# tangih/video-matting

Measured on AMD Instinct MI355X. Metric: alpha-mattes/sec at 1920×1080, 1/2/4/8 MI355X + achieved HBM GB/s, higher is better.
Workload: dtype bf16; 1 GPU; unet.UNetVideo forward (20 3x3 convs, 3.233 TFLOP/frame), 1920x1080 7-ch NHWC; height=1080, width=1920, launch=hip-graph replay, parallelism=frame-parallel dp1

## Files before the change

### video-matting_amd/csrc/conv3x3.hip

```cpp

#include <cstring>
#include <initializer_list>

#include "conv_dispatch.h"

namespace vm {


struct TileOrigin {
  int h0, w0;
  float rcp_w, rcp_h;
};

__device__ __forceinline__ TileOrigin tile_origin(long m0, int H, int W) {
  TileOrigin o;
  const long q = m0 / W;
  o.w0 = (int)(m0 - q * W);
  o.h0 = (int)(q % H);
  o.rcp_w = __builtin_amdgcn_rcpf((float)W);
  o.rcp_h = __builtin_amdgcn_rcpf((float)H);
  return o;
}

__device__ __forceinline__ int fast_div(int t, int d, float rcp) {
// ... 454 lines not shown
        float bsv[4] = {0.f, 0.f, 0.f, 0.f}, scv[4] = {1.f, 1.f, 1.f, 1.f}, shv[4] = {0.f, 0.f, 0.f, 0.f};
#pragma unroll
        for (int j = 0; j < 4; ++j) {
          const int co = min(n0 + wn * 64 + col + j, a.cout - 1);
          if (a.bias) bsv[j] = a.bias[co];
          if (a.scale) scv[j] = a.scale[co];
          if (a.shift) shv[j] = a.shift[co];
        }
#pragma unroll
        for (int fp = 0; fp < FP; ++fp) {
          const int row = wm * C::TPM + fp * 16 + (lane & 15);
          float4 v;
          float* vv = reinterpret_cast<float*>(&v);
#pragma unroll
          for (int j = 0; j < 4; ++j) {
            float tv = (acc[fc][fp][j] + bsv[j]) * scv[j] + shv[j];
            if (a.act == VM_ACT_RELU) tv = tv > 0.f ? tv : 0.f;
            else if (a.act == VM_ACT_SIGMOID) tv = sigmoid_precise(tv);
            vv[j] = tv;
          }
          *reinterpret_cast<float4*>(stg + row * SROW + col) = v;
        }
      }
    }
    __syncthreads();
    const int nb = n0 + sl * 64;
    if (a.y_dtype == VM_BF16) {
      uint16_t* Y = reinterpret_cast<uint16_t*>(a.y) + a.y_coff;
      for (int idx = tid; idx < BM * 8; idx += NT) {
        const int rr = idx >> 3, cc = idx & 7;
        const long p = m0 + rr;
        const int co = nb + cc * 8;
        if (p >= a.M || co >= a.cout) continue;
        const float* src = stg + rr * SROW + cc * 8;
        uint16_t* dst = Y + p * (long)a.y_cstride + co;
        if (a.y_vec && co + 8 <= a.cout) *reinterpret_cast<uint4*>(dst) = Chunk<uint16_t>::pack(src);
        else
          for (int j = 0; j < 8 && co + j < a.cout; ++j) dst[j] = f2bf(src[j]);
      }
    } else {
      float* Y = reinterpret_cast<float*>(a.y) + a.y_coff;
      for (int idx = tid; idx < BM * 16; idx += NT) {
        const int rr = idx >> 4, cc = idx & 15;
        const long p = m0 + rr;
        const int co = nb + cc * 4;
        if (p >= a.M || co >= a.cout) continue;
        const float* src = stg + rr * SROW + cc * 4;
        float* dst = Y + p * (long)a.y_cstride + co;
        if (a.y_vec && co + 4 <= a.cout) *reinterpret_cast<float4*>(dst) = *reinterpret_cast<const float4*>(src);
        else
          for (int j = 0; j < 4 && co + j < a.cout; ++j) dst[j] = src[j];
      }
    }
  }
}

thread_local char g_last_kernel[128];
ConvOptions g_opt;
template <typename T>
static const char* tname() { return sizeof(T) == 2 ? "unsigned short" : "float"; }

template <typename T, int BM, int BN>
static int launch_mfma(ConvArgs& a, hipStream_t st) {
  constexpr int lds = mfma_lds_bytes<BM, BN>();
  static bool attr_set = false;
  if (!attr_set) {
    hipError_t e = hipFuncSetAttribute(reinterpret_cast<const void*>(&conv3x3_mfma<T, BM, BN>),
                                       hipFuncAttributeMaxDynamicSharedMemorySize, lds);
    if (e != hipSuccess) return fail(VM_EHIP, "hipFuncSetAttribute: %s", hipGetErrorString(e));
    attr_set = true;
  }
  a.nk = a.K_pad / (128 / (int)sizeof(T));
  a.tiles_n = (a.cout + BN - 1) / BN;
  a.tiles_total = (int)((a.M + BM - 1) / BM) * a.tiles_n;
  snprintf(g_last_kernel, sizeof g_last_kernel, "vm::conv3x3_mfma<%s, %d, %d>", tname<T>(), BM, BN);
  hipLaunchKernelGGL((conv3x3_mfma<T, BM, BN>), dim3(a.tiles_total), dim3(256), lds, st, a);
  return check_launch("conv3x3_mfma");
}

template <typename T, int RB, int BM, int BN, int WM, int WN, int S, bool FAST>
static int launch_glds(ConvArgs& a, hipStream_t st) {
  using C = GldsCfg<T, RB, BM, BN, WM, WN, S>;
  static bool attr_set = false;
  if (!attr_set) {
    hipError_t e = hipFuncSetAttribute(reinterpret_cast<const void*>(&conv3x3_glds<T, RB, BM, BN, WM, WN, S, FAST>),
                                       hipFuncAttributeMaxDynamicSharedMemorySize, C::LDS);
    if (e != hipSuccess) return fail(VM_EHIP, "hipFuncSetAttribute(glds): %s", hipGetErrorString(e));
    attr_set = true;
  }
  const int bke = RB / (int)sizeof(T);
  a.nk = (FAST && RB == 64) ? a.ng : a.K_pad / bke;
  a.tiles_n = (a.cout + BN - 1) / BN;
  a.tiles_total = (int)((a.M + BM - 1) / BM) * a.tiles_n;
  snprintf(g_last_kernel, sizeof g_last_kernel, "vm::conv3x3_glds<%s, %d, %d, %d, %d, %d, %d, %s>", tname<T>(), RB,
           BM, BN, WM, WN, S, FAST ? "true" : "false");
  hipLaunchKernelGGL((conv3x3_glds<T, RB, BM, BN, WM, WN, S, FAST>), dim3(a.tiles_total), dim3(C::NT), C::LDS, st,
                     a);
  return check_launch("conv3x3_glds");
}

template <typename T, bool FAST>
static int dispatch_glds(ConvArgs& a, hipStream_t st) {
  if constexpr (sizeof(T) == 2) {
    if (a.cout > 128) {
      if (g_opt.glds_rb == 64) return launch_glds<T, 64, 256, 256, 2, 4, 4, FAST>(a, st);
      return launch_glds<T, 128, 256, 256, 2, 4, 2, FAST>(a, st);
    }
  }
  if (a.cout > 64) return launch_glds<T, 64, 256, 128, 4, 2, 6, FAST>(a, st);
  return launch_glds<T, 64, 512, 64, 8, 1, 4, FAST>(a, st);
}

template <typename T>
static int dispatch_mfma(ConvArgs& a, hipStream_t st, int cin = 0) {
  if (sizeof(T) == 4 && g_opt.softmax_kernel != 0 && g_opt.conv_kernel != 1 && g_opt.conv_kernel != 2 && cin > 0 && cin <= 8 &&
      a.cin_pad == 8 && !a.chunk_major && a.x_src_c <= 0 && a.y_dtype == VM_F32 && a.y_vec && a.act == VM_ACT_SOFTMAX &&
      a.cout == 64 && a.K_pad == 96 && a.x_cstride % 4 == 0 && a.x_coff % 4 == 0 &&
      reinterpret_cast<uintptr_t>(a.x) % 16 == 0)
    return launch_first_softmax_f32(a, cin, st);
  if (sizeof(T) == 2 && g_opt.softmax_kernel != 0 && g_opt.conv_kernel != 1 && g_opt.conv_kernel != 2 && a.cin_pad == 8 &&
      !a.chunk_major && a.x_src_c <= 0 && a.y_dtype == VM_F32 && a.y_vec && a.act == VM_ACT_SOFTMAX && a.cout == 64 &&
      a.K_pad == 128)
    return launch_first_softmax(a, st);
  if (sizeof(T) == 2 && g_opt.conv_kernel != 1 && g_opt.conv_kernel != 2 && a.cin_pad == 8 && !a.chunk_major && a.x_src_c <= 0 &&
      a.y_dtype == VM_BF16 && a.y_vec && a.act != VM_ACT_SOFTMAX && (a.cout & 7) == 0 && a.K_pad == 128)
    return launch_first(a, st);
  if ((g_opt.conv_kernel == 0 || g_opt.conv_kernel == 3) && patch_ok(a, sizeof(T))) return dispatch_patch(a, st);
  if (g_opt.conv_kernel != 1 && a.act != VM_ACT_SOFTMAX && a.x_src_c <= 0) {
    const int bm = a.cout > 64 ? 256 : 512;
    const long tiles = ((a.M + bm - 1) / bm) * ((a.cout + 255) / 256);
    const bool wide = sizeof(T) == 2 && a.cout > 128;
    if (g_opt.conv_kernel == 2 || (wide && tiles >= g_opt.conv_min_tiles))
      return a.chunk_major ? dispatch_glds<T, true>(a, st) : dispatch_glds<T, false>(a, st);
  }
  if (a.cout <= 64) return launch_mfma<T, 256, 64>(a, st);
  return launch_mfma<T, 128, 128>(a, st);
}

static const OptDef conv_options[] = {
    {"conv_kernel", &g_opt.conv_kernel, OPT_RANGE, 2, {0, 3}},
    {"softmax_kernel", &g_opt.softmax_kernel, OPT_RANGE, 2, {0, 6}},
    {"softmax_blocks", &g_opt.softmax_blocks, OPT_RANGE, 2, {1, 1 << 20}},
    {"head_th", &g_opt.head_th, OPT_SET, 2, {8, 16}},
    {"softmax_f32p", &g_opt.softmax_f32p, OPT_RANGE, 2, {0, 7}},
    {"cband", &g_opt.cband, OPT_RANGE, 2, {0, 2}},
    {"ngroup", &g_opt.ngroup, OPT_RANGE, 2, {0, 64}},
    {"cband_bytes", &g_opt.cband_bytes, OPT_ANY},
    {"rows_kernel", &g_opt.rows_kernel, OPT_SET, 4, {0, 1, 8, 16}},
    {"pack_tiled", &g_opt.pack_tiled, OPT_ANY},
    {"persist_half", &g_opt.persist_half, OPT_ANY},
    {"rows_up", &g_opt.rows_up, OPT_ANY},
    {"rows_min_cin", &g_opt.rows_min_cin, OPT_ANY},
    {"rows_min_blocks", &g_opt.rows_min_blocks, OPT_ANY},
    {"thin_rounds", &g_opt.thin_rounds, OPT_RANGE, 2, {0, 64}},
    {"pack_frames", &g_opt.pack_frames, OPT_RANGE, 2, {0, 1}},
    {"up_skip", &g_opt.up_skip, OPT_RANGE, 2, {0, 1}},
    {"src_span_limit", &g_opt.src_span_limit, OPT_RANGE, 2, {1, 0x7ffffff0L}},
    {"thin_blocks", &g_opt.thin_blocks, OPT_ANY},
    {"thin_th", &g_opt.thin_th, OPT_SET, 3, {4, 8, 16}},
    {"conv_prio", &g_opt.conv_prio, OPT_RANGE, 2, {0, 1}},
    {"thin_twalk", &g_opt.thin_twalk, OPT_RANGE, 2, {0, 1}},
    {"thin_rowreuse", &g_opt.thin_rowreuse, OPT_RANGE, 2, {0, 1}},
    {"thin_dma", &g_opt.thin_dma, OPT_RANGE, 2, {0, 4}},
    {"thin_dma_rounds", &g_opt.thin_dma_rounds, OPT_RANGE, 2, {1, 64}},
    {"narrowin_kernel", &g_opt.narrowin_kernel, OPT_RANGE, 2, {0, 1}},
    {"thin_kernel", &g_opt.thin_kernel, OPT_RANGE, 2, {0, 1}},
    {"conv_min_tiles", &g_opt.conv_min_tiles, OPT_ANY},
#ifdef VM_STUDY
    {"patch_cfg", &g_opt.patch_cfg, OPT_RANGE, 2, {0, 31}},
    {"patch_ablate", &g_opt.patch_ablate, OPT_ANY},
    {"softmax_abl", &g_opt.softmax_abl, OPT_ANY},
    {"patch_rowslot", &g_opt.patch_rowslot, OPT_RANGE, 2, {0, 1}},
    {"pair_strip_abl", &g_opt.pair_strip_abl, OPT_ANY},
    {"pair_kernel", &g_opt.pair_kernel, OPT_RANGE, 2, {0, 1}},
    {"pair_kernel", &g_opt.pair_kernel, OPT_RANGE, 2, {10, 18}},
#else
    {"patch_cfg", &g_opt.patch_cfg, OPT_SET, 5, {0, 19, 22, 25, 30}, " (other tilings: the study build)"},
    {"pair_kernel", &g_opt.pair_kernel, OPT_RANGE, 2, {0, 1}, " (ablations: the study build)"},
#endif
    {"pair_xin_wide", &g_opt.pair_xin_wide, OPT_RANGE, 2, {0, 1}},
    {"border_ks", &g_opt.border_ks, OPT_SET, 3, {1, 2, 4}},
    {"border_fuse", &g_opt.border_fuse, OPT_RANGE, 2, {0, 2}},
    {"patch_repi", &g_opt.patch_repi, OPT_RANGE, 2, {0, 1}},
    {"persist_rounds", &g_opt.persist_rounds, OPT_RANGE, 2, {0, 64}, " (0: any grid)"},
    {"persist_up_rounds", &g_opt.persist_up_rounds, OPT_RANGE, 2, {0, 64}, " (0: any grid)"},
    {"persist_all", &g_opt.persist_all, OPT_RANGE, 2, {0, 2}},
    {"persist_rot", &g_opt.persist_rot, OPT_RANGE, 2, {0, 2}},
    {"up_skip_mask", &g_opt.up_skip_mask, OPT_RANGE, 2, {0, 3}},
    {"patch_persist", &g_opt.patch_persist, OPT_RANGE, 2, {0, 1}},
    {"pair_strip_pin", &g_opt.pair_strip_pin, OPT_RANGE, 2, {0, 1}},
    {"pair_strip", &g_opt.pair_strip, OPT_RANGE, 2, {0, 1}},
    {"head_kernel", &g_opt.head_kernel, OPT_RANGE, 2, {0, 2}},
    {"splitk_tiles", &g_opt.splitk_tiles, OPT_ANY},
    {"glds_rb", &g_opt.glds_rb, OPT_SET, 2, {64, 128}},
    {nullptr},
};
}

using namespace vm;

static int set_from(const OptDef* t, const char* key, long value) {
  char want[160] = "";
  const char* note = "";
  for (; t->key; ++t) {
    if (strcmp(key, t->key)) continue;
    bool ok = t->kind == OPT_ANY || (t->kind == OPT_RANGE && value >= t->v[0] && value <= t->v[1]);
    for (int i = 0; t->kind == OPT_SET && i < t->n; ++i) ok = ok || value == t->v[i];
    if (ok) {
      *t->value = value;
      return VM_OK;
    }
    size_t len = strlen(want);
    if (len) len += snprintf(want + len, sizeof want - len, " or ");
    if (t->kind == OPT_RANGE) snprintf(want + len, sizeof want - len, "%ld..%ld", t->v[0], t->v[1]);
    for (int i = 0; t->kind == OPT_SET && i < t->n && len < sizeof want; ++i)
      len += snprintf(want + len, sizeof want - len, i == 0 ? "%ld" : i + 1 < t->n ? ", %ld" : " or %ld", t->v[i]);
    if (t->note) note = t->note;
  }
  return want[0] ? fail(VM_EINVAL, "set_option: %s must be %s%s", key, want, note) : 1;
}

extern "C" int vm_set_option(const char* key, long value) {
  if (!key) return fail(VM_EINVAL, "set_option: NULL key");
  for (const OptDef* t : {conv_options, bn_options, train_options, wgrad_options, flow_options}) {
    const int rc = set_from(t, key, value);
    if (rc != 1) return rc;
  }
  return fail(VM_EINVAL, "set_option: unknown key '%s'", key);
}

extern "C" const char* vm_conv3x3_last_kernel(void) { return g_last_kernel; }

static int conv_impl(const ConvCall& c);

extern "C" int vm_conv3x3_nhwc(const vm_tensor* x, const void* packed, int cin, int cout, const float* bias,
                               const float* scale, const float* shift, int act, vm_tensor* y, void* stream) {
  return conv_impl({x, packed, cin, cout, bias, scale, shift, act, y, stream});
}

extern "C" int vm_conv3x3_sources_nhwc(const vm_tensor* x, int nsrc, long src_stride, const void* packed, int cin,
                                       int cout, const float* bias, const float* scale, const float* shift, int act,
                                       vm_tensor* y, void* stream) {
  if (nsrc < 1 || (nsrc > 1 && src_stride <= 0)) return fail(VM_EINVAL, "conv3x3_sources: nsrc %d stride %ld", nsrc,
                                                            src_stride);
  ConvCall c{x, packed, cin, cout, bias, scale, shift, act, y, stream};
  c.nsrc = nsrc;
  c.src_stride = src_stride;
  return conv_impl(c);
}

extern "C" int vm_conv3x3_pool_nhwc(const vm_tensor* x, const void* packed, int cin, int cout, const float* bias,
                                    const float* scale, const float* shift, int act, vm_tensor* y, vm_tensor* ypool,
                                    void* stream) {
  if (!valid_tensor(ypool) || !y) return fail(VM_EINVAL, "conv3x3_pool: invalid pool tensor");
  if (ypool->n != y->n || ypool->h != (y->h + 1) / 2 || ypool->w != (y->w + 1) / 2 || ypool->c != cout ||
      ypool->dtype != y->dtype)
    return fail(VM_EINVAL, "conv3x3_pool: pool output must be [n, ceil(h/2), ceil(w/2), cout] in the output dtype");
  ConvCall c{x, packed, cin, cout, bias, scale, shift, act, y, stream};
  c.yp = ypool;
  return conv_impl(c);
}

extern "C" int vm_conv3x3_head_acc_nhwc(const vm_tensor* x, const void* packed, int cin, const float* bias,
                                        const float* y_acc, vm_tensor* y, float* alpha, void* stream) {
  if (!y_acc) return fail(VM_EINVAL, "conv3x3_head_acc: y_acc is NULL");
  ConvCall c{x, packed, cin, 1, bias, nullptr, nullptr, VM_ACT_NONE, y, stream};
  c.y2 = alpha;
  c.y_acc = y_acc;
  return conv_impl(c);
}

extern "C" int vm_conv3x3_head_acc_ex_nhwc(const vm_tensor* x, const void* packed, int cin, const float* bias,
                                           const float* scale, const float* shift, const float* y_acc, vm_tensor* y,
                                           float* alpha, void* stream) {
  ConvCall c{x, packed, cin, 1, bias, scale, shift, VM_ACT_NONE, y, stream};
  c.y2 = alpha;
  c.y_acc = y_acc;
  return conv_impl(c);
}

extern "C" int vm_conv3x3_split3_nhwc(const vm_tensor* x, const void* packed, int cin, int cout, const float* bias,
                                      const float* scale, const float* shift, int act, vm_tensor* y, int y_slab,
                                      vm_tensor* ypool, int pool_slab, int* overflow, void* work, size_t work_bytes,
                                      void* stream) {
  if (!x || !y || !valid_tensor(y, true) || (ypool && !valid_tensor(ypool, true)))
    return fail(VM_EINVAL, "conv3x3_split3: invalid tensor");
  SplitOut so{y_slab > 0 ? y_slab : y->cstride / 2, 0, overflow};
  if (cout % 8 || !split3_view_ok(y, so.yslab, cout))
    return fail(VM_EUNSUPPORTED, "conv3x3_split3: y must be an fp16 view of cout %% 8 == 0 channels inside the first "
                                 "of two (or three) slabs of S %% 8 == 0 channels, 16-byte aligned");
  if (ypool) {
    so.pslab = pool_slab > 0 ? pool_slab : ypool->cstride / 2;
    if (!split3_view_ok(ypool, so.pslab, cout) || ypool->n != y->n || ypool->h != (y->h + 1) / 2 ||
        ypool->w != (y->w + 1) / 2 || ypool->c != cout)
      return fail(VM_EINVAL, "conv3x3_split3: pool view must be [n, ceil(h/2), ceil(w/2), cout] in the split layout");
  }
  ConvCall c{x, packed, cin, cout, bias, scale, shift, act, y, stream};
  c.yp = ypool;
  c.work = work;
  c.work_bytes = work_bytes;
  c.so = &so;
  return conv_impl(c);
}

extern "C" int vm_conv3x3_head_partial_nhwc(const vm_tensor* x, const void* packed, int cin, const float* bias,
                                            const float* scale, const float* shift, int act, vm_tensor* y,
                                            float* alpha, const float* partial, void* stream) {
  if (!partial) return fail(VM_EINVAL, "conv3x3_head_partial: partial is NULL");
  ConvCall c{x, packed, cin, 1, bias, scale, shift, act, y, stream};
  c.y2 = alpha;
  c.head_part = partial;
  return conv_impl(c);
}

extern "C" int vm_conv3x3_head_nhwc(const vm_tensor* x, const void* packed, int cin, const float* bias,
                                    const float* scale, const float* shift, int act, vm_tensor* y, float* alpha,
                                    void* stream) {
  ConvCall c{x, packed, cin, 1, bias, scale, shift, act, y, stream};
  c.y2 = alpha;
  return conv_impl(c);
}

static int conv_impl(const ConvCall& c) {
// ... 138 lines not shown
```

### video-matting_amd/csrc/conv_common.h

```cpp
#pragma once

#include <type_traits>

#include "vm_common.h"

namespace vm {

struct ConvArgs {
  const void* x;
  int x_cstride, x_coff, H, W;
  long M;
  int cin_pad, K9, nk;
  int chunk_major, ng;
  const void* w;
  int K_pad, cout, cout_pad;
  const float* bias;
  const float* scale;
  const float* shift;
  int act;
  void* y;
  int y_cstride, y_coff, y_dtype, y_vec;
  int tiles_n, tiles_total;
  void* py;
  int py_cstride, py_coff;
  int up, up_cout;
  const void* w1;
  const float* bias1;
  int x_f32, x_c;
  int x_src_c;
  long x_src_stride;
  int ksplit;
  float* part;
  float* hd;
  const float* hw;
  int hw_cin, hw_coff, y_skip;
  int vstride, vW;
  int repi;
  int prot;
  int upmask;
  int cband;
  int ngroup;
  int twalk;
  int seg;
  int prio;
  void* y1;
  int y1_cstride, y1_coff;
  int halfskip;
  int f16;
  int ysplit, psplit;
  int* ovf;
  int xalias;
  int bwant, bfuse, bblocks, bframes, bK_pad;
  const void* bw;
};

template <int I, int N, typename F>
__device__ __forceinline__ void static_for(F&& f) {
  if constexpr (I < N) {
    f(std::integral_constant<int, I>{});
    static_for<I + 1, N>(f);
  }
}

template <typename P>
__device__ __forceinline__ P* uniform_ptr(P* p) {
  const uint64_t v = reinterpret_cast<uint64_t>(p);
  const uint32_t lo = __builtin_amdgcn_readfirstlane((uint32_t)v), hi = __builtin_amdgcn_readfirstlane((uint32_t)(v >> 32));
  return reinterpret_cast<P*>(((uint64_t)hi << 32) | lo);
}

__device__ __forceinline__ long src_chan(const ConvArgs& a, int c) {
  if (a.xalias > 0 && c >= 2 * a.xalias) c -= a.xalias;
  if (a.x_src_c <= 0) return c;
  const int s = c / a.x_src_c;
  return (long)s * a.x_src_stride + (c - s * a.x_src_c);
}

template <int GE>
__device__ __forceinline__ void k_to_tap(const ConvArgs& a, int k, int& tap, int& c) {
  if (a.chunk_major) {
    const int g = k / GE;
    if (g < a.ng) {
      const int cc = g / 9;
      tap = g - cc * 9;
      c = cc * GE + (k - g * GE);
    } else {
      tap = 9;
      c = 0;
    }
  } else if (k < a.K9) {
    tap = k / a.cin_pad;
    c = k - tap * a.cin_pad;
  } else {
    tap = 9;
    c = 0;
  }
}

template <int RB>
__device__ __forceinline__ int swz(int row, int chunk) {
  if constexpr (RB == 128) return row * 128 + ((chunk ^ ((row >> 1) & 7)) << 4);
  else return row * 64 + ((chunk ^ (((row >> 2) & 1) << 1)) << 4);
}

__device__ __forceinline__ int swz2(int row, int chunk) { return row * 64 + ((chunk ^ ((row >> 1) & 3)) << 4); }

template <typename T>
__device__ __forceinline__ void mma16(const uint4& a, const uint4& b, f32x4& c);

template <>
__device__ __forceinline__ void mma16<uint16_t>(const uint4& a, const uint4& b, f32x4& c) {
  c = __builtin_amdgcn_mfma_f32_16x16x32_bf16(__builtin_bit_cast(bf16x8, a), __builtin_bit_cast(bf16x8, b), c, 0, 0,
                                               0);
}

template <>
__device__ __forceinline__ void mma16<f16_t>(const uint4& a, const uint4& b, f32x4& c) {
  c = __builtin_amdgcn_mfma_f32_16x16x32_f16(__builtin_bit_cast(f16x8, a), __builtin_bit_cast(f16x8, b), c, 0, 0, 0);
}

template <>
__device__ __forceinline__ void mma16<float>(const uint4& a, const uint4& b, f32x4& c) {
  c = __builtin_amdgcn_mfma_f32_16x16x4f32(__uint_as_float(a.x), __uint_as_float(b.x), c, 0, 0, 0);
  c = __builtin_amdgcn_mfma_f32_16x16x4f32(__uint_as_float(a.y), __uint_as_float(b.y), c, 0, 0, 0);
  c = __builtin_amdgcn_mfma_f32_16x16x4f32(__uint_as_float(a.z), __uint_as_float(b.z), c, 0, 0, 0);
  c = __builtin_amdgcn_mfma_f32_16x16x4f32(__uint_as_float(a.w), __uint_as_float(b.w), c, 0, 0, 0);
}

__device__ __forceinline__ bool split3h_chunk(const float* v, uint4& H, uint4& L) {
  typedef _Float16 h2_t __attribute__((ext_vector_type(2)));
  typedef float f2_t __attribute__((ext_vector_type(2)));
  uint32_t wh[4], wl[4];
  bool ovf = false;
#pragma unroll
  for (int i = 0; i < 4; ++i) {
    const f2_t x = {v[2 * i], v[2 * i + 1]};
    const h2_t h = __builtin_convertvector(x, h2_t);
    wh[i] = __builtin_bit_cast(uint32_t, h);
    const f2_t r = {v[2 * i] - (float)h[0], v[2 * i + 1] - (float)h[1]};
    wl[i] = __builtin_bit_cast(uint32_t, __builtin_convertvector(r, h2_t));
    ovf |= !(fabsf(v[2 * i]) < 65520.f) || !(fabsf(v[2 * i + 1]) < 65520.f);
  }
  H = make_uint4(wh[0], wh[1], wh[2], wh[3]);
  L = make_uint4(wl[0], wl[1], wl[2], wl[3]);
  return ovf;
}

__device__ __forceinline__ int xcd_tile(int b, int nwg) {
  const int q = nwg >> 3, r8 = nwg & 7, xcd = b & 7;
  return (xcd < r8 ? xcd * (q + 1) : r8 * (q + 1) + (xcd - r8) * q) + (b >> 3);
}

template <typename T>
__device__ __forceinline__ __amdgpu_buffer_rsrc_t x_rsrc(const ConvArgs& a, long xbase) {
  const T* Xb = reinterpret_cast<const T*>(a.x) + a.x_coff + xbase * (long)a.x_cstride;
  return __builtin_amdgcn_make_buffer_rsrc(const_cast<T*>(Xb), 0, 0x7ffffff0, 0x00020000);
}
template <typename T>
__device__ __forceinline__ __amdgpu_buffer_rsrc_t w_rsrc(const ConvArgs& a, int n0) {
  const T* Wb = reinterpret_cast<const T*>(a.w) + (long)n0 * a.K_pad;
  const uint32_t bytes = (uint32_t)((long)(a.cout_pad - n0) * a.K_pad * (long)sizeof(T));
  return __builtin_amdgcn_make_buffer_rsrc(const_cast<T*>(Wb), 0, bytes, 0x00020000);
}

__device__ __forceinline__ int ring_row(const ConvArgs& a, int phase) { return !a.bfuse ? -1 : (phase >> 1) ? a.H - 1 : 0; }
__device__ __forceinline__ int ring_col(const ConvArgs& a, int phase) { return !a.bfuse ? -1 : (phase & 1) ? a.W - 1 : 0; }

constexpr int OOB = (int)0x80000000;
constexpr int OOB_INL = (int)0xC0800000;

typedef __attribute__((address_space(3))) void* lds_ptr_t;

__device__ __forceinline__ uint32_t lds_addr(const char* p) {
  return (uint32_t)(uintptr_t)(lds_ptr_t)(p);
}

__device__ __forceinline__ void glds16(__amdgpu_buffer_rsrc_t rsrc, uint32_t lds_dst, int voffset) {
  unsigned keep;
  asm volatile(
      "s_mov_b32 %0, m0\n\t"
      "s_mov_b32 m0, %2\n\t"
      "s_nop 0\n\t"
      "buffer_load_dwordx4 %1, %3, 0 offen lds\n\t"
      "s_mov_b32 m0, %0"
      : "=&s"(keep)
      : "v"(voffset), "s"(lds_dst), "s"(rsrc)
      : "memory");
}

__device__ __forceinline__ void wait_vm(int n) {
#define VM_W(N) \
  case N:       \
    asm volatile("s_waitcnt vmcnt(" #N ")" ::: "memory"); \
    break;
  switch (n) {
    VM_W(0) VM_W(1) VM_W(2) VM_W(3) VM_W(4) VM_W(5) VM_W(6) VM_W(7) VM_W(8) VM_W(9) VM_W(10) VM_W(11) VM_W(12)
    VM_W(13) VM_W(14) VM_W(15) VM_W(16) VM_W(17) VM_W(18) VM_W(19) VM_W(20) VM_W(21) VM_W(22) VM_W(23) VM_W(24)
    VM_W(25) VM_W(26) VM_W(27) VM_W(28) VM_W(29) VM_W(30) VM_W(31) VM_W(32) VM_W(33) VM_W(34) VM_W(35) VM_W(36)
    VM_W(37) VM_W(38) VM_W(39) VM_W(40) VM_W(41) VM_W(42) VM_W(43) VM_W(44) VM_W(45) VM_W(46) VM_W(47) VM_W(48)
    VM_W(49) VM_W(50) VM_W(51) VM_W(52) VM_W(53) VM_W(54) VM_W(55) VM_W(56) VM_W(57) VM_W(58) VM_W(59) VM_W(60)
    VM_W(61) VM_W(62) VM_W(63)
    default: asm volatile("s_waitcnt vmcnt(0)" ::: "memory");
  }
#undef VM_W
}

// ... 9 lines not shown
```

### video-matting_amd/csrc/conv_dispatch.h

```cpp
#pragma once

#include "conv_common.h"

namespace vm {

struct ConvOptions {
  long conv_kernel = 0;
  long conv_min_tiles = 128;
  long glds_rb = 128;
  long head_kernel = 0;
  long head_th = 16;
  long patch_cfg = 0;
  long softmax_abl = 0;
  long patch_rowslot = 1;
  long patch_ablate = 0;
  long rows_kernel = 1;
  long rows_min_blocks = 400;
  long rows_up = 0;
  long rows_min_cin = 64;
  long src_span_limit = 0x7ffffff0L;
  long pair_strip = 1;
  long pair_kernel = 0;
  long pair_xin_wide = 1;
  long pair_strip_abl = 0;
  long pair_strip_pin = 1;
  long conv_prio = 0;

  long border_ks = 1;
  long border_fuse = 2;
  long up_skip_mask = 3;
  long patch_repi = 1;
  long cband = 0;
  long cband_bytes = 4L << 20;
  long ngroup = 0;
  long pack_tiled = 1;
  long up_skip = 1;
  long patch_persist = 1;
  long persist_rounds = 2;
  long persist_up_rounds = 6;
  long persist_all = 0;
  long persist_rot = 0;
  long persist_half = 1;
  long splitk_tiles = 512;
  long pack_frames = 1;

  long thin_kernel = 1;
  long narrowin_kernel = 1;
  long thin_th = 8, thin_blocks = 512;
  long thin_rounds = 1;
  long thin_dma = 0, thin_dma_rounds = 1;
  long thin_rowreuse = 1;
  long thin_twalk = 1;

  long softmax_kernel = 6;
  long softmax_blocks = 2048;
  long softmax_f32p = 4;
};
extern ConvOptions g_opt;

extern thread_local char g_last_kernel[128];

struct PackGeom {
  int cin_pad, ge, K9, K_pad, cout_pad, chunk_major, ng;
};

inline PackGeom geom(int cin, int cout, int dtype) {
  PackGeom g;
  g.ge = 64 / elem_bytes(dtype);
  g.cin_pad = (cin + 7) / 8 * 8;
  g.K9 = 9 * g.cin_pad;
  g.chunk_major = g.cin_pad % g.ge == 0;
  g.ng = g.chunk_major ? g.K9 / g.ge : 0;
  g.K_pad = (g.K9 + 2 * g.ge - 1) / (2 * g.ge) * (2 * g.ge);
  g.cout_pad = (cout + 63) / 64 * 64;
  return g;
}

inline void fill_geom(ConvArgs& a, const PackGeom& g) {
  a.cin_pad = g.cin_pad;
  a.K9 = g.K9;
  a.chunk_major = g.chunk_major;
  a.ng = g.ng;
  a.K_pad = g.K_pad;
  a.cout_pad = g.cout_pad;
}

struct SplitOut {
  int yslab, pslab;
  int* ovf;
};

struct ConvCall {
  const vm_tensor* x;
  const void* packed;
  int cin, cout;
  const float* bias;
  const float* scale;
  const float* shift;
  int act;
  vm_tensor* y;
  void* stream;
  const vm_tensor* yp = nullptr;
  float* y2 = nullptr;
  int nsrc = 0;
  long src_stride = 0;
  void* work = nullptr;
  size_t work_bytes = 0;
  const float* head_part = nullptr;
  const float* y_acc = nullptr;
  const SplitOut* so = nullptr;
};

inline bool split3_view_ok(const vm_tensor* t, int slab, int c) {
  return t->dtype == VM_F16 && view16_ok(t) && slab > 0 && slab % 8 == 0 && t->coff + c <= slab && 2 * slab <= t->cstride;
}

bool patch_ok(const ConvArgs& a, size_t tsize);
int dispatch_patch(ConvArgs& a, hipStream_t st);
int splitk_plan(long n, int h, int w, int cin_pad, int cout);
int launch_splitk_reduce(const ConvArgs& a, hipStream_t st);
int launch_patch_first(ConvArgs& a, hipStream_t st);
bool thin_ok(int dt, const PackGeom& g, int cout, int x_src_c, int act, const vm_tensor* x);
bool narrowin_ok(const ConvArgs& a, const PackGeom& g, int cout, int act, const vm_tensor* x, const vm_tensor* y);
int launch_narrowin(ConvArgs& a, long n, const PackGeom& g, hipStream_t st);
int thin_splitk_plan(long n, int h, int w, int cin_pad);
int dispatch_thin(ConvArgs& a, long n, hipStream_t st);
bool rows_ok(const ConvArgs& a);
int launch_rows(ConvArgs& a, hipStream_t st, int cfg);
int launch_first(ConvArgs& a, hipStream_t st);
int launch_first_softmax(ConvArgs& a, hipStream_t st);
int launch_first_softmax_f32(ConvArgs& a, int cin, hipStream_t st);
int dispatch_head(const ConvCall& c, const PackGeom& g, int xalias, long M, hipStream_t st);

}
```

### video-matting_amd/csrc/conv_rows.hip

```cpp
#include <type_traits>

#include "conv_dispatch.h"

namespace vm {

template <int TH_>
struct RowsCfg {
  static constexpr int R = 4;
  static constexpr int TH = TH_, TW = 32, BM = TH * TW, BN = 64;
  static constexpr int RG = TH / R, CG = 8 / RG;
  static constexpr int CW = BN / CG, FC = CW / 16;
  static constexpr int PW = TW + 2, PPIX = (TH + 2) * PW;
  static constexpr int XP = (PPIX + 15) / 16, XPW = (XP + 7) / 8;
  static constexpr int PB = XP * 1024;
  static constexpr int WP = 9 * BN / 16, WPW = (WP + 7) / 8;
  static constexpr int WB = 9 * BN * 64;
  static constexpr int JUNK = 2 * PB + 2 * WB;
  static constexpr int LDS = JUNK + 1024;
  static_assert(RG * CG == 8 && FC >= 1, "8 waves");
  static_assert(LDS <= 163840, "one CU's LDS");
};

template <int FC>
constexpr int row_mfmas(int ir) {
// ... 72 lines not shown
    r.n = st / (th * tw);
    const int srem = st - r.n * th * tw;
    r.r0 = (srem / tw) * TH;
    r.c0 = (srem - (srem / tw) * tw) * C::TW;
    r.n0 = nt * C::BN;
    r.n = __builtin_amdgcn_readfirstlane(r.n);
    r.r0 = __builtin_amdgcn_readfirstlane(r.r0);
    r.c0 = __builtin_amdgcn_readfirstlane(r.c0);
    r.n0 = __builtin_amdgcn_readfirstlane(r.n0);
    return r;
  };

  const int lrow = lane >> 2, lpos = lane & 3;
  int xgeo[XPW];
#pragma unroll
  for (int i = 0; i < XPW; ++i) {
    const int piece = wave + i * 8;
    const int row = piece * 16 + lrow;
    const int lq = (swz<64>(row, lpos) - row * 64) >> 4;
    const int pr = row / PW, pc = row - pr * PW;
    xgeo[i] = row < C::PPIX ? (pr << 16) | (pc << 8) | lq : -1;
  }
  int woff[WPW];
#pragma unroll
  for (int i = 0; i < WPW; ++i) {
    const int piece = wave + i * 8;
    const int tap = piece / (C::BN / 16);
    const int row = (piece - tap * (C::BN / 16)) * 16 + lrow;
    const int lq = (swz<64>(row, lpos) - row * 64) >> 4;
    woff[i] = (row * a.K_pad + lq * 8) * 2 + tap * 64;
  }
  const uint32_t lds0 = __builtin_amdgcn_readfirstlane(lds_addr(smem));
  const int ccap = a.up ? a.up_cout : a.cout;
  float2* const ctab = reinterpret_cast<float2*>(smem + C::LDS);
  for (int c = tid; c < ccap; c += 512) {
    const float sc = a.scale ? a.scale[c] : 1.f;
    ctab[c] = make_float2(sc, (a.bias ? a.bias[c] : 0.f) * sc + (a.shift ? a.shift[c] : 0.f));
  }
  auto issue_x = [&](const RowTile& tt, bool real, int g, int buf, auto i0c, auto i1c) __attribute__((always_inline)) {
    constexpr int i0 = decltype(i0c)::value, i1 = decltype(i1c)::value;
    const T* xb = uniform_ptr(reinterpret_cast<const T*>(a.x) + a.x_coff + (long)tt.n * H * W * cs);
    const __amdgpu_buffer_rsrc_t xrs = __builtin_amdgcn_make_buffer_rsrc(const_cast<T*>(xb), 0, 0x7ffffff0, 0x00020000);
    const int coff = (int)src_chan(a, g * 32) * 2;
#pragma unroll
    for (int i = i0; i < i1; ++i) {
      const bool piece_ok = wave + i * 8 < C::XP;
      int h = tt.r0 - 1 + (xgeo[i] >> 16), w = tt.c0 - 1 + ((xgeo[i] >> 8) & 255);
      if (a.up) {
        h = min(h, H - 1);
        w = min(w, W - 1);
      }
      const bool ok = real && xgeo[i] >= 0 && (unsigned)h < (unsigned)H && (unsigned)w < (unsigned)W;
      glds16(xrs, __builtin_amdgcn_readfirstlane(lds0 + (piece_ok ? 2 * C::WB + buf * C::PB + (wave + i * 8) * 1024 : C::JUNK)),
             ok ? ((h * W + w) * cs + (xgeo[i] & 255) * 8) * 2 + coff : OOB);
    }
  };
  auto issue_w = [&](int n0, bool real, int g, int buf, auto i0c, auto i1c) __attribute__((always_inline)) {
    constexpr int i0 = decltype(i0c)::value, i1 = decltype(i1c)::value;
    const T* wb = uniform_ptr(reinterpret_cast<const T*>(a.w) + (long)n0 * a.K_pad);
    const uint32_t wbytes = __builtin_amdgcn_readfirstlane((uint32_t)((long)(a.cout_pad - n0) * a.K_pad * 2));
    const __amdgpu_buffer_rsrc_t wrs = __builtin_amdgcn_make_buffer_rsrc(const_cast<T*>(wb), 0, wbytes, 0x00020000);
#pragma unroll
    for (int i = i0; i < i1; ++i) {
      const bool piece_ok = wave + i * 8 < C::WP;
      glds16(wrs, __builtin_amdgcn_readfirstlane(lds0 + (piece_ok ? buf * C::WB + (wave + i * 8) * 1024 : C::JUNK)),
             real && piece_ok ? woff[i] + g * 576 : OOB);
    }
  };
  auto sync = [&](auto nconst) __attribute__((always_inline)) {
    asm volatile("s_waitcnt vmcnt(%0)" ::"n"(decltype(nconst)::value) : "memory");
    asm volatile("s_waitcnt lgkmcnt(0)" ::: "memory");
    __builtin_amdgcn_s_barrier();
    asm volatile("" ::: "memory");
  };

  const int ck = lane >> 4, col = lane & 15;
  const int pbase = rg * R * PW + col;
  int pxa[8];
#pragma unroll
  for (int v = 0; v < 8; ++v)
    pxa[v] = 2 * C::WB + pbase * 64 + ((ck ^ ((((pbase & 7) + v) >> 2) & 1) * 2) << 4);
  int wa[FC];
#pragma unroll
  for (int f = 0; f < FC; ++f) wa[f] = swz<64>(cg * C::CW + f * 16 + col, ck);

  typedef uint4 WRow[3][FC];
  auto ldw = [&](WRow& w, const int buf, const int kh) __attribute__((always_inline)) {
#pragma unroll
    for (int kw = 0; kw < 3; ++kw)
#pragma unroll
      for (int f = 0; f < FC; ++f)
        w[kw][f] = *reinterpret_cast<const uint4*>(smem + wa[f] + buf * C::WB + (kh * 3 + kw) * (C::BN * 64));
  };
  typedef uint4 XRow[3][2];
  auto ldx = [&](XRow& x, const int buf, const int ir) __attribute__((always_inline)) {
#pragma unroll
    for (int kw = 0; kw < 3; ++kw)
#pragma unroll
      for (int pf = 0; pf < 2; ++pf) {
        const int K = ir * PW + pf * 16 + kw;
        x[kw][pf] = *reinterpret_cast<const uint4*>(smem + pxa[K & 7] + K * 64 + buf * C::PB);
      }
  };

  f32x4 acc[R][FC][2];
#pragma unroll
  for (int o = 0; o < R; ++o)
#pragma unroll
    for (int f = 0; f < FC; ++f)
#pragma unroll
      for (int pf = 0; pf < 2; ++pf) acc[o][f][pf] = f32x4{0.f, 0.f, 0.f, 0.f};

  WRow w0, w1, w2, w3;
  auto row_mma = [&](const int ir, const XRow& x, const WRow& k2) __attribute__((always_inline)) {
#pragma unroll
    for (int kw = 0; kw < 3; ++kw)
#pragma unroll
      for (int kh = 0; kh < 3; ++kh) {
        const int o = ir - kh;
        if (o < 0 || o >= R) continue;
#pragma unroll
        for (int f = 0; f < FC; ++f)
#pragma unroll
          for (int pf = 0; pf < 2; ++pf) {
            const uint4& wv = kh == 0 ? w0[kw][f] : (kh == 1 ? w1[kw][f] : k2[kw][f]);
            mma16<MT>(wv, x[kw][pf], acc[o][f][pf]);
          }
      }
  };

  bool ovf = false;
  auto epilogue = [&](const RowTile& tt) __attribute__((always_inline)) {
    const int phase = a.up ? tt.n0 / a.up_cout : 0;
    const int cb = tt.n0 - phase * a.up_cout;
    const int YH = a.up ? 2 * H : H, YW = a.up ? 2 * W : W;
    T* yb = uniform_ptr(reinterpret_cast<T*>(a.y) + a.y_coff + (long)tt.n * YH * YW * a.y_cstride);
    const __amdgpu_buffer_rsrc_t yrs = __builtin_amdgcn_make_buffer_rsrc(yb, 0, 0x7ffffff0, 0x00020000);
    const int PH = (H + 1) >> 1, PWo = (W + 1) >> 1;
    T* pbp = uniform_ptr(a.py ? reinterpret_cast<T*>(a.py) + a.py_coff + (long)tt.n * PH * PWo * a.py_cstride : nullptr);
    const __amdgpu_buffer_rsrc_t prs = __builtin_amdgcn_make_buffer_rsrc(pbp, 0, 0x7ffffff0, 0x00020000);
    float mul[FC][4], add[FC][4];
#pragma unroll
    for (int f = 0; f < FC; ++f)
#pragma unroll
      for (int j = 0; j < 4; ++j) {
        const float2 t = ctab[min(cb + cg * C::CW + f * 16 + 4 * ck + j, ccap - 1)];
        mul[f][j] = t.x;
        add[f][j] = t.y;
      }
    auto pack4 = [](const float (&v)[4]) __attribute__((always_inline)) {
      return make_uint2(bf16x2_bits(v[0], v[1]), bf16x2_bits(v[2], v[3]));
    };
    const int c16 = (ck & 1) ? 2 + (ck >> 1) : ck >> 1;
#pragma unroll
    for (int pf = 0; pf < 2; ++pf) {
      const int c = tt.c0 + pf * 16 + col;
      float v[R][FC][4];
#pragma unroll
      for (int o = 0; o < R; ++o) {
        const int r = tt.r0 + rg * R + o;
#pragma unroll
        for (int f = 0; f < FC; ++f)
#pragma unroll
          for (int j = 0; j < 4; ++j) {
            float t = fmaf(acc[o][f][pf][j], mul[f][j], add[f][j]);
            if (a.act == VM_ACT_RELU) t = fmaxf(t, 0.f);
            else if (a.act == VM_ACT_SIGMOID) t = sigmoid_precise(t);
            v[o][f][j] = t;
          }
        const int pix = a.up ? (2 * r + (phase >> 1)) * YW + 2 * c + (phase & 1) : r * W + c;
        if constexpr (SPL) {
          typedef __attribute__((ext_vector_type(4))) unsigned u4_t;
          typedef __attribute__((ext_vector_type(2))) unsigned u2_t;
          const int S2 = a.ysplit * 2;
          const bool y3 = 3 * a.ysplit <= a.y_cstride;
          uint2 hq[FC], lq[FC];
          bool o2 = false;
#pragma unroll
          for (int f = 0; f < FC; ++f) o2 |= split4h(v[o][f], hq[f], lq[f]);
          if constexpr (FC == 2) {
            const int chan = cb + cg * C::CW + c16 * 8;
            const bool ok = r < H && c < W && chan < ccap;
            ovf |= ok && o2;
            const int off = ok ? (pix * a.y_cstride + chan) * 2 : OOB;
            __builtin_amdgcn_raw_buffer_store_b128(__builtin_bit_cast(u4_t, chunk_pair(lq[0], lq[1])), yrs, off, 0, 0);
            const uint4 dh = chunk_pair(hq[0], hq[1]);
            __builtin_amdgcn_raw_buffer_store_b128(__builtin_bit_cast(u4_t, dh), yrs, ok ? off + S2 : OOB, 0, 0);
            if (y3) __builtin_amdgcn_raw_buffer_store_b128(__builtin_bit_cast(u4_t, dh), yrs, ok ? off + 2 * S2 : OOB, 0, 0);
          } else {
#pragma unroll
            for (int f = 0; f < FC; ++f) {
              const int chan = cb + cg * C::CW + f * 16 + 4 * ck;
              const bool ok = r < H && c < W && chan < ccap;
              ovf |= ok && o2;
              const int off = ok ? (pix * a.y_cstride + chan) * 2 : OOB;
              __builtin_amdgcn_raw_buffer_store_b64(__builtin_bit_cast(u2_t, lq[f]), yrs, off, 0, 0);
              __builtin_amdgcn_raw_buffer_store_b64(__builtin_bit_cast(u2_t, hq[f]), yrs, ok ? off + S2 : OOB, 0, 0);
              if (y3) __builtin_amdgcn_raw_buffer_store_b64(__builtin_bit_cast(u2_t, hq[f]), yrs, ok ? off + 2 * S2 : OOB, 0, 0);
            }
          }
        } else if constexpr (FC == 2) {
          const int chan = cb + cg * C::CW + c16 * 8;
          const uint4 d = chunk_pair(pack4(v[o][0]), pack4(v[o][1]));
          const bool ok = r < H && c < W && chan < ccap;
          __builtin_amdgcn_raw_buffer_store_b128(__builtin_bit_cast(__attribute__((ext_vector_type(4))) unsigned, d),
                                                 yrs, ok ? (pix * a.y_cstride + chan) * 2 : OOB, 0, 0);
        } else {
#pragma unroll
          for (int f = 0; f < FC; ++f) {
            const int chan = cb + cg * C::CW + f * 16 + 4 * ck;
            const bool ok = r < H && c < W && chan < ccap;
            __builtin_amdgcn_raw_buffer_store_b64(
                __builtin_bit_cast(__attribute__((ext_vector_type(2))) unsigned, pack4(v[o][f])), yrs,
                ok ? (pix * a.y_cstride + chan) * 2 : OOB, 0, 0);
          }
        }
      }
      if (a.py) {
#pragma unroll
        for (int op = 0; op < R / 2; ++op) {
          const int r = tt.r0 + rg * R + 2 * op;
          const bool v0 = r < H && c < W, v1 = r + 1 < H && c < W;
          float m[FC][4];
#pragma unroll
          for (int f = 0; f < FC; ++f)
#pragma unroll
            for (int j = 0; j < 4; ++j) {
              float t = v0 ? v[2 * op][f][j] : -INFINITY;
              if (v1) t = fmaxf(t, v[2 * op + 1][f][j]);
              const float u = __int_as_float(__builtin_amdgcn_mov_dpp(__float_as_int(t), 0xB1, 0xF, 0xF, false));
              m[f][j] = fmaxf(t, u);
            }
          const int pr = r >> 1, pc = c >> 1;
          const bool pok = (col & 1) == 0 && pr < PH && pc < PWo;
          if constexpr (SPL) {
            typedef __attribute__((ext_vector_type(4))) unsigned u4_t;
            typedef __attribute__((ext_vector_type(2))) unsigned u2_t;
            const int P2 = a.psplit * 2;
            const bool p3 = 3 * a.psplit <= a.py_cstride;
            uint2 hq[FC], lq[FC];
#pragma unroll
            for (int f = 0; f < FC; ++f) split4h(m[f], hq[f], lq[f]);
            if constexpr (FC == 2) {
              const int chan = tt.n0 + cg * C::CW + c16 * 8;
              const int off = pok && chan < a.cout ? ((pr * PWo + pc) * a.py_cstride + chan) * 2 : OOB;
              const uint4 dh = chunk_pair(hq[0], hq[1]);
              __builtin_amdgcn_raw_buffer_store_b128(__builtin_bit_cast(u4_t, chunk_pair(lq[0], lq[1])), prs, off, 0, 0);
              __builtin_amdgcn_raw_buffer_store_b128(__builtin_bit_cast(u4_t, dh), prs, off == OOB ? OOB : off + P2, 0, 0);
              if (p3)
                __builtin_amdgcn_raw_buffer_store_b128(__builtin_bit_cast(u4_t, dh), prs, off == OOB ? OOB : off + 2 * P2, 0,
                                                       0);
            } else {
#pragma unroll
              for (int f = 0; f < FC; ++f) {
                const int chan = tt.n0 + cg * C::CW + f * 16 + 4 * ck;
                const int off = pok && chan < a.cout ? ((pr * PWo + pc) * a.py_cstride + chan) * 2 : OOB;
                __builtin_amdgcn_raw_buffer_store_b64(__builtin_bit_cast(u2_t, lq[f]), prs, off, 0, 0);
                __builtin_amdgcn_raw_buffer_store_b64(__builtin_bit_cast(u2_t, hq[f]), prs, off == OOB ? OOB : off + P2, 0, 0);
                if (p3)
                  __builtin_amdgcn_raw_buffer_store_b64(__builtin_bit_cast(u2_t, hq[f]), prs, off == OOB ? OOB : off + 2 * P2,
                                                        0, 0);
              }
            }
          } else if constexpr (FC == 2) {
            const int chan = tt.n0 + cg * C::CW + c16 * 8;
            const uint4 d = chunk_pair(pack4(m[0]), pack4(m[1]));
            __builtin_amdgcn_raw_buffer_store_b128(__builtin_bit_cast(__attribute__((ext_vector_type(4))) unsigned, d),
                                                   prs, pok && chan < a.cout ? ((pr * PWo + pc) * a.py_cstride + chan) * 2 : OOB,
                                                   0, 0);
          } else {
#pragma unroll
            for (int f = 0; f < FC; ++f) {
              const int chan = tt.n0 + cg * C::CW + f * 16 + 4 * ck;
              __builtin_amdgcn_raw_buffer_store_b64(
                  __builtin_bit_cast(__attribute__((ext_vector_type(2))) unsigned, pack4(m[f])), prs,
                  pok && chan < a.cout ? ((pr * PWo + pc) * a.py_cstride + chan) * 2 : OOB, 0, 0);
            }
          }
        }
      }
    }
  };

  int s = 0, k = 0, g = 0;
  RowTile t0 = tile_of(0), t1 = tile_of(ntile > 1 ? 1 : 0), t2 = tile_of(ntile > 2 ? 2 : 0);
  using Z = std::integral_constant<int, 0>;
  using NX = std::integral_constant<int, XPW>;
  using NW = std::integral_constant<int, WPW>;
  auto issue_step = [&](int d, bool wts, int buf, auto i0, auto i1) __attribute__((always_inline)) {
    const int gd = g + d;
    const int dk = (gd >= nch ? 1 : 0) + (gd >= 2 * nch ? 1 : 0);
    const int gg = gd - dk * nch;
    const int m1 = dk >= 1, m2 = dk >= 2;
    RowTile tt;
    tt.n = t0.n + m1 * (t1.n - t0.n) + m2 * (t2.n - t1.n);
    tt.r0 = t0.r0 + m1 * (t1.r0 - t0.r0) + m2 * (t2.r0 - t1.r0);
    tt.c0 = t0.c0 + m1 * (t1.c0 - t0.c0) + m2 * (t2.c0 - t1.c0);
    tt.n0 = t0.n0 + m1 * (t1.n0 - t0.n0) + m2 * (t2.n0 - t1.n0);
    const bool real = k + dk < ntile;
    if (wts) issue_w(tt.n0, real, gg, buf, i0, i1);
    else issue_x(tt, real, gg, buf, i0, i1);
  };
  using I = std::integral_constant<int, 0>;
  issue_w(t0.n0, true, 0, 0, I{}, NW{});
  issue_x(t0, true, 0, 0, I{}, NX{});
  sync(Z{});
  issue_step(1, true, 1, I{}, NW{});
  ldw(w0, 0, 0);
  ldw(w1, 0, 1);
  ldw(w2, 0, 2);

  auto step = [&](auto bconst) __attribute__((always_inline)) {
    constexpr int b = decltype(bconst)::value;
    static_assert(R == 4, "the row schedule below is written for 4-row waves");
    WRow& k2 = b == 0 ? w2 : w3;
    WRow& n2 = b == 0 ? w3 : w2;
    XRow xa, xb;
    ldx(xa, b, 0);
    ldx(xb, b, 1);
    issue_step(1, false, b ^ 1, I{}, std::integral_constant<int, 2>{});
    row_mma(0, xa, k2);
    ldx(xa, b, 2);
    issue_step(1, false, b ^ 1, std::integral_constant<int, 2>{}, std::integral_constant<int, 4>{});
    row_mma(1, xb, k2);
    ldx(xb, b, 3);
    issue_step(1, false, b ^ 1, std::integral_constant<int, 4>{}, NX{});
    row_mma(2, xa, k2);
    ldx(xa, b, 4);
    row_mma(3, xb, k2);
    sched_rows<FC, 12, 6, 6, 6, 0>();
    __builtin_amdgcn_sched_barrier(0);
    sync(NX{});
    __builtin_amdgcn_sched_barrier(0);
    ldx(xb, b, 5);
    issue_step(2, true, b, I{}, std::integral_constant<int, 2>{});
    ldw(w0, b ^ 1, 0);
    issue_step(2, true, b, std::integral_constant<int, 2>{}, std::integral_constant<int, 4>{});
    ldw(n2, b ^ 1, 2);
    row_mma(4, xa, k2);
    issue_step(2, true, b, std::integral_constant<int, 4>{}, NW{});
    ldw(w1, b ^ 1, 1);
    row_mma(5, xb, k2);
    sched_tail<FC>();
    __builtin_amdgcn_sched_barrier(0);
    sync(NW{});
    if (g == nch - 1) {
      epilogue(t0);
#pragma unroll
      for (int o = 0; o < R; ++o)
#pragma unroll
        for (int f = 0; f < FC; ++f)
#pragma unroll
          for (int pf = 0; pf < 2; ++pf) acc[o][f][pf] = f32x4{0.f, 0.f, 0.f, 0.f};
      g = 0;
      ++k;
      t0 = t1;
      t1 = t2;
      if (k + 2 < ntile) t2 = tile_of(k + 2);
    } else {
      ++g;
    }
    ++s;
  };
  while (s < S) {
    step(std::integral_constant<int, 0>{});
    if (s < S) step(std::integral_constant<int, 1>{});
  }
  asm volatile("s_waitcnt vmcnt(0)" ::: "memory");
  if (SPL && ovf && a.ovf) *a.ovf = 1;
}

bool rows_ok(const ConvArgs& a) {
  const long img_in = (long)a.H * a.W * a.x_cstride * 2;
  const long img_out = (long)(a.up ? 4 : 1) * a.H * a.W * a.y_cstride * 2;
  const bool yok = a.f16 ? a.ysplit > 0 : a.y_dtype == VM_BF16;
  return a.chunk_major && a.cin_pad % 32 == 0 && yok && a.y_vec && (a.cout & 7) == 0 &&
         a.act != VM_ACT_SOFTMAX && a.ksplit <= 1 && (a.x_src_c <= 0 || a.x_src_c % 32 == 0) &&
         (!a.up || a.up_cout % 64 == 0) && img_in < 0x7ffffff0L && img_out < 0x7ffffff0L &&
         (!a.py || (a.py_cstride % 8 == 0 && a.py_coff % 8 == 0)) &&
         RowsCfg<16>::LDS + 8 * (a.up ? a.up_cout : a.cout) <= 163840;
}

static int g_num_cu = 0;

template <int TH, bool SPL>
static int launch_th(ConvArgs& a, hipStream_t st) {
  using C = RowsCfg<TH>;
  const int lds = C::LDS + 8 * (a.up ? a.up_cout : a.cout);
  if (lds > 163840) return fail(VM_EUNSUPPORTED, "conv3x3_rows: %d output channels overflow LDS", a.cout);
  static bool attr_set = false;
  if (!attr_set) {
    hipError_t e = hipFuncSetAttribute(reinterpret_cast<const void*>(&conv3x3_rows<TH, SPL>),
                                       hipFuncAttributeMaxDynamicSharedMemorySize, 163840);
    if (e != hipSuccess) return fail(VM_EHIP, "hipFuncSetAttribute(rows): %s", hipGetErrorString(e));
    attr_set = true;
  }
  if (!g_num_cu) {
    int dev = 0, n = 0;
    if (hipGetDevice(&dev) != hipSuccess || hipDeviceGetAttribute(&n, hipDeviceAttributeMultiprocessorCount, dev) != hipSuccess || n <= 0)
      return fail(VM_EHIP, "conv3x3_rows: cannot read the CU count");
    g_num_cu = n;
  }
  const long N = a.M / ((long)a.H * a.W);
  const long sp = N * ((a.H + TH - 1) / TH) * ((a.W + C::TW - 1) / C::TW);
  a.tiles_n = (a.cout + C::BN - 1) / C::BN;
  if (sp * a.tiles_n > 0x7fffffffL) return fail(VM_EUNSUPPORTED, "conv3x3: too many tiles");
  a.tiles_total = (int)(sp * a.tiles_n);
  a.prio = (int)g_opt.conv_prio;
  long grid = g_num_cu < a.tiles_total ? g_num_cu : a.tiles_total;
  grid = (grid + 7) / 8 * 8;
  snprintf(g_last_kernel, sizeof g_last_kernel, SPL ? "vm::conv3x3_rows<%d, true>" : "vm::conv3x3_rows<%d>", TH);
  hipLaunchKernelGGL((conv3x3_rows<TH, SPL>), dim3(grid), dim3(512), lds, st, a);
  return check_launch("conv3x3_rows");
}

int launch_rows(ConvArgs& a, hipStream_t st, int cfg) {
  if (a.f16) {
    if (a.ysplit <= 0) return fail(VM_EUNSUPPORTED, "conv3x3_rows: fp16 operands need the split output");
    return cfg == 8 ? launch_th<8, true>(a, st) : launch_th<16, true>(a, st);
  }
  if (cfg == 8) return launch_th<8, false>(a, st);
  return launch_th<16, false>(a, st);
}

}
```

Baseline: 336.8 frames/s.

## Split rows-kernel epilogue into paired retires overlapped with final k-step

Adds a retire path for the TH=16 non-split rows conv kernel. It writes output rows in pairs, and the first pair is stored inside the last K-chunk step: before the weight loads for lower waves, and before the final sync for upper waves. Doing this spreads the epilogue stores and the fused 2x2 max-pool stores across the pipeline instead of stalling everything at the end of a tile. It relaxes the sync wait counts to account for the extra in-flight stores. It also adds study-only ablation switches that disable the stores or the epilogue. The cost is added register pressure and schedule complexity in the hot loop.

```diff
diff --git a/video-matting_amd/csrc/conv3x3.hip b/video-matting_amd/csrc/conv3x3.hip
--- a/video-matting_amd/csrc/conv3x3.hip
+++ b/video-matting_amd/csrc/conv3x3.hip
@@ -630,6 +630,7 @@
     {"rows_up", &g_opt.rows_up, OPT_ANY},
     {"rows_min_cin", &g_opt.rows_min_cin, OPT_ANY},
     {"rows_min_blocks", &g_opt.rows_min_blocks, OPT_ANY},
+    {"rows_retire", &g_opt.rows_retire, OPT_RANGE, 2, {0, 1}},
     {"thin_rounds", &g_opt.thin_rounds, OPT_RANGE, 2, {0, 64}},
     {"pack_frames", &g_opt.pack_frames, OPT_RANGE, 2, {0, 1}},
     {"up_skip", &g_opt.up_skip, OPT_RANGE, 2, {0, 1}},
@@ -647,6 +648,7 @@
 #ifdef VM_STUDY
     {"patch_cfg", &g_opt.patch_cfg, OPT_RANGE, 2, {0, 31}},
     {"patch_ablate", &g_opt.patch_ablate, OPT_ANY},
+    {"rows_ablate", &g_opt.rows_ablate, OPT_RANGE, 2, {0, 2}},
     {"softmax_abl", &g_opt.softmax_abl, OPT_ANY},
     {"patch_rowslot", &g_opt.patch_rowslot, OPT_RANGE, 2, {0, 1}},
     {"pair_strip_abl", &g_opt.pair_strip_abl, OPT_ANY},
diff --git a/video-matting_amd/csrc/conv_common.h b/video-matting_amd/csrc/conv_common.h
--- a/video-matting_amd/csrc/conv_common.h
+++ b/video-matting_amd/csrc/conv_common.h
@@ -52,6 +52,7 @@
   int xalias;
   int bwant, bfuse, bblocks, bframes, bK_pad;
   const void* bw;
+  int retire, rabl;
 };
 
 template <int I, int N, typename F>
diff --git a/video-matting_amd/csrc/conv_dispatch.h b/video-matting_amd/csrc/conv_dispatch.h
--- a/video-matting_amd/csrc/conv_dispatch.h
+++ b/video-matting_amd/csrc/conv_dispatch.h
@@ -18,6 +18,8 @@
   long rows_min_blocks = 400;
   long rows_up = 0;
   long rows_min_cin = 64;
+  long rows_retire = 1;
+  long rows_ablate = 0;
   long src_span_limit = 0x7ffffff0L;
   long pair_strip = 1;
   long pair_kernel = 0;
diff --git a/video-matting_amd/csrc/conv_rows.hip b/video-matting_amd/csrc/conv_rows.hip
--- a/video-matting_amd/csrc/conv_rows.hip
+++ b/video-matting_amd/csrc/conv_rows.hip
@@ -248,6 +248,11 @@
       return make_uint2(bf16x2_bits(v[0], v[1]), bf16x2_bits(v[2], v[3]));
     };
     const int c16 = (ck & 1) ? 2 + (ck >> 1) : ck >> 1;
+#ifdef VM_STUDY
+    const bool wr = a.rabl != 2;
+#else
+    constexpr bool wr = true;
+#endif
 #pragma unroll
     for (int pf = 0; pf < 2; ++pf) {
       const int c = tt.c0 + pf * 16 + col;
@@ -298,7 +303,7 @@
         } else if constexpr (FC == 2) {
           const int chan = cb + cg * C::CW + c16 * 8;
           const uint4 d = chunk_pair(pack4(v[o][0]), pack4(v[o][1]));
-          const bool ok = r < H && c < W && chan < ccap;
+          const bool ok = wr && r < H && c < W && chan < ccap;
           __builtin_amdgcn_raw_buffer_store_b128(__builtin_bit_cast(__attribute__((ext_vector_type(4))) unsigned, d),
                                                  yrs, ok ? (pix * a.y_cstride + chan) * 2 : OOB, 0, 0);
         } else {
@@ -328,7 +333,7 @@
               m[f][j] = fmaxf(t, u);
             }
           const int pr = r >> 1, pc = c >> 1;
-          const bool pok = (col & 1) == 0 && pr < PH && pc < PWo;
+          const bool pok = wr && (col & 1) == 0 && pr < PH && pc < PWo;
           if constexpr (SPL) {
             typedef __attribute__((ext_vector_type(4))) unsigned u4_t;
             typedef __attribute__((ext_vector_type(2))) unsigned u2_t;
@@ -374,6 +379,80 @@
             }
           }
         }
+      }
+    }
+  };
+
+  constexpr bool RET = !SPL && TH == 16;
+  auto st16 = [](const __amdgpu_buffer_rsrc_t rs, const uint4 d, const int off) __attribute__((always_inline)) {
+    __builtin_amdgcn_raw_buffer_store_b128(__builtin_bit_cast(__attribute__((ext_vector_type(4))) unsigned, d), rs, off, 0, 0);
+  };
+  auto retire_pair = [&](const RowTile& tt, const int op) __attribute__((always_inline)) {
+    int ln = lane;
+    asm volatile("" : "+v"(ln));
+    const int ck = ln >> 4, col = ln & 15;
+    int H = a.H, W = a.W, ycs = a.y_cstride, yco = a.y_coff, ccap_ = ccap, act = a.act;
+    const int cout = a.cout;
+    asm volatile("" : "+s"(H), "+s"(W), "+s"(ycs), "+s"(yco), "+s"(ccap_), "+s"(act));
+    const int c16 = (ck & 1) ? 2 + (ck >> 1) : ck >> 1;
+    const bool relu = act == VM_ACT_RELU;
+    T* yb = uniform_ptr(reinterpret_cast<T*>(a.y) + yco + (long)tt.n * H * W * ycs);
+    const __amdgpu_buffer_rsrc_t yrs = __builtin_amdgcn_make_buffer_rsrc(yb, 0, 0x7ffffff0, 0x00020000);
+    float mul[FC][4], add[FC][4];
+#pragma unroll
+    for (int f = 0; f < FC; ++f) {
+      const float4* cp = reinterpret_cast<const float4*>(ctab + min(tt.n0 + cg * C::CW + f * 16 + 4 * ck, ccap_ - 4));
+      const float4 c0 = cp[0], c1 = cp[1];
+      mul[f][0] = c0.x, add[f][0] = c0.y, mul[f][1] = c0.z, add[f][1] = c0.w;
+      mul[f][2] = c1.x, add[f][2] = c1.y, mul[f][3] = c1.z, add[f][3] = c1.w;
+    }
+    const int chan = tt.n0 + cg * C::CW + c16 * 8;
+    const int r = tt.r0 + rg * R + 2 * op;
+    float v[2][2][FC][4];
+#pragma unroll
+    for (int i = 0; i < 2; ++i) {
+      const int o = 2 * op + i;
+#pragma unroll
+      for (int pf = 0; pf < 2; ++pf) {
+        const int c = tt.c0 + pf * 16 + col;
+#pragma unroll
+        for (int f = 0; f < FC; ++f) {
+#pragma unroll
+          for (int j = 0; j < 4; ++j) {
+            const float t = fmaf(acc[o][f][pf][j], mul[f][j], add[f][j]);
+            v[i][pf][f][j] = relu ? fmaxf(t, 0.f) : t;
+          }
+        }
+        const uint2 lo = make_uint2(bf16x2_bits(v[i][pf][0][0], v[i][pf][0][1]), bf16x2_bits(v[i][pf][0][2], v[i][pf][0][3]));
+        const uint2 hi = make_uint2(bf16x2_bits(v[i][pf][FC - 1][0], v[i][pf][FC - 1][1]),
+                                    bf16x2_bits(v[i][pf][FC - 1][2], v[i][pf][FC - 1][3]));
+        st16(yrs, chunk_pair(lo, hi), r + i < H && c < W && chan < ccap_ ? (((r + i) * W + c) * ycs + chan) * 2 : OOB);
+      }
+    }
+    if (a.py) {
+      const int PH = (H + 1) >> 1, PWo = (W + 1) >> 1;
+      const int pcs = a.py_cstride, pco = a.py_coff;
+      T* pbp = uniform_ptr(reinterpret_cast<T*>(a.py) + pco + (long)tt.n * PH * PWo * pcs);
+      const __amdgpu_buffer_rsrc_t prs = __builtin_amdgcn_make_buffer_rsrc(pbp, 0, 0x7ffffff0, 0x00020000);
+#pragma unroll
+      for (int pf = 0; pf < 2; ++pf) {
+        const int c = tt.c0 + pf * 16 + col;
+        const bool v0 = r < H && c < W, v1 = r + 1 < H && c < W;
+        float m[FC][4];
+#pragma unroll
+        for (int f = 0; f < FC; ++f)
+#pragma unroll
+          for (int j = 0; j < 4; ++j) {
+            float t = v0 ? v[0][pf][f][j] : -INFINITY;
+            if (v1) t = fmaxf(t, v[1][pf][f][j]);
+            const float u = __int_as_float(__builtin_amdgcn_mov_dpp(__float_as_int(t), 0xB1, 0xF, 0xF, false));
+            m[f][j] = fmaxf(t, u);
+          }
+        const int pr = r >> 1, pc = c >> 1;
+        const bool pok = (col & 1) == 0 && pr < PH && pc < PWo;
+        const uint2 lo = make_uint2(bf16x2_bits(m[0][0], m[0][1]), bf16x2_bits(m[0][2], m[0][3]));
+        const uint2 hi = make_uint2(bf16x2_bits(m[FC - 1][0], m[FC - 1][1]), bf16x2_bits(m[FC - 1][2], m[FC - 1][3]));
+        st16(prs, chunk_pair(lo, hi), pok && chan < cout ? ((pr * PWo + pc) * pcs + chan) * 2 : OOB);
       }
     }
   };
@@ -406,6 +485,7 @@
   ldw(w1, 0, 1);
   ldw(w2, 0, 2);
 
+  const int rmode = RET && a.retire ? (wave >= 4 ? 2 : 1) : 0;
   auto step = [&](auto bconst) __attribute__((always_inline)) {
     constexpr int b = decltype(bconst)::value;
     static_assert(R == 4, "the row schedule below is written for 4-row waves");
@@ -428,6 +508,11 @@
     __builtin_amdgcn_sched_barrier(0);
     sync(NX{});
     __builtin_amdgcn_sched_barrier(0);
+    int rm = rmode;
+    if constexpr (RET) asm volatile("" : "+s"(rm));
+    if constexpr (RET) {
+      if (rm == 1 && g == nch - 1) retire_pair(t0, 0);
+    }
     ldx(xb, b, 5);
     issue_step(2, true, b, I{}, std::integral_constant<int, 2>{});
     ldw(w0, b ^ 1, 0);
@@ -439,9 +524,22 @@
     row_mma(5, xb, k2);
     sched_tail<FC>();
     __builtin_amdgcn_sched_barrier(0);
-    sync(NW{});
+    if (rm && g == nch - 1) {
+      if (rm == 2) retire_pair(t0, 0);
+      if (a.py) sync(std::integral_constant<int, WPW + 6>{});
+      else sync(std::integral_constant<int, WPW + 4>{});
+    } else {
+      sync(NW{});
+    }
     if (g == nch - 1) {
-      epilogue(t0);
+      if (rm) {
+        retire_pair(t0, 1);
+      } else {
+#ifdef VM_STUDY
+        if (a.rabl != 1)
+#endif
+        epilogue(t0);
+      }
 #pragma unroll
       for (int o = 0; o < R; ++o)
 #pragma unroll
@@ -503,6 +601,12 @@
   if (sp * a.tiles_n > 0x7fffffffL) return fail(VM_EUNSUPPORTED, "conv3x3: too many tiles");
   a.tiles_total = (int)(sp * a.tiles_n);
   a.prio = (int)g_opt.conv_prio;
+  a.retire = g_opt.rows_retire && TH == 16 && !SPL && !a.up && a.act != VM_ACT_SIGMOID;
+  a.rabl = 0;
+#ifdef VM_STUDY
+  a.rabl = (int)g_opt.rows_ablate;
+  if (a.rabl) a.retire = 0;
+#endif
   long grid = g_num_cu < a.tiles_total ? g_num_cu : a.tiles_total;
   grid = (grid + 7) / 8 * 8;
   snprintf(g_last_kernel, sizeof g_last_kernel, SPL ? "vm::conv3x3_rows<%d, true>" : "vm::conv3x3_rows<%d>", TH);
```

Result: faster. 357.6 frames/s, median of 6 (+6.2%).
